# Ryan-D-Gast/ivp

Measured on AMD Instinct MI355X. Metric: accepted RK steps/sec (aggregate), batched CR3BP DOPRI5 @ rtol=1e-6, higher is better.
Workload: dtype f64; 1 GPU; C2: 100k independent 6-state CR3BP trajectories (perturbed Arenstorf orbits, one period), DOPRI5 rtol=1e-6 atol=1e-9; one step = whole batch integrated to t_end; trajectories_total=100000, trajectories_per_gpu=100000, fp_mode=strict, chunk_attempts=64, parallelism=dp1 (independent shards)

## Files before the change

ivp_amd/csrc/bdf_core.h:

```cpp
#pragma once
#ifndef __HIPCC_RTC__
#include "rk_core.h"
#endif

namespace IVP_NS {

constexpr int BDF_MAXO = 5;
#define IVP_BDF_ORDER_SHIFT 4
#define IVP_BDF_NEQ_SHIFT 8
#define IVP_BDF_LU_CURRENT 0x1000u
#define IVP_BDF_PENDING 0x2000u

#if defined(IVP_PHASE_PROF) && defined(__HIP_DEVICE_COMPILE__)
__device__ __forceinline__ unsigned long long *ivp_phase_lds()
{
    __shared__ unsigned long long t[18];
    return t;
}
__device__ __forceinline__ bool ivp_phase_leader()
{
    return __builtin_amdgcn_mbcnt_hi(__builtin_amdgcn_read_exec_hi(), __builtin_amdgcn_mbcnt_lo(__builtin_amdgcn_read_exec_lo(), 0u)) == 0u;
}
__device__ __forceinline__ void ivp_phase_mark(int k)
{
// ... 756 lines not shown
    a.hlamb[js] = S.pending_factor;
    a.bdf_piv[js] = S.piv;
    a.flags[js] = (S.flags & ~IVP_F_FIRSTOUT) | (L.flags & IVP_F_FIRSTOUT);
    a.status[js] = S.status;
    a.nfev[js] += S.d_nfev; a.njev[js] += S.d_njev; a.nlu[js] += S.d_nlu;
    a.nstep[js] += S.d_nstep; a.naccpt[js] += S.d_naccpt; a.nrejct[js] += S.d_nrejct;
    if (FULL) {
        a.next_idx[js] = L.next_idx; a.n_filled[js] = L.n_filled; a.n_log[js] = L.n_log;
        a.n_seg[js] = L.n_seg; a.t_last[js] = L.t_last;
    }
    status_out = S.status;
    return it;
}

template <class R, int FULL>
IVP_HD int32_t radau_init_body(const IvpKArgs &a, uint32_t j);
template <class R, int FULL>
IVP_HD uint32_t radau_chunk_body(const IvpKArgs &a, uint32_t j, int32_t &status_out);

template <int M, class R, int FULL>
IVP_HD int32_t any_init_body(const IvpKArgs &a, uint32_t j)
{
    if constexpr (M == M_BDF) return bdf_init_body<R, FULL>(a, j);
    else if constexpr (M == M_RADAU) return radau_init_body<R, FULL>(a, j);
    else return init_body<M, R, FULL>(a, j);
}
template <int M, class R, int FULL, bool CTL = false>
IVP_HD uint32_t any_chunk_body(const IvpKArgs &a, uint32_t j, int32_t &status_out)
{
    if constexpr (M == M_BDF) return bdf_chunk_body<R, FULL>(a, j, status_out);
    else if constexpr (M == M_RADAU) return radau_chunk_body<R, FULL>(a, j, status_out);
    else return chunk_body<M, R, FULL, CTL>(a, j, status_out);
}

}
```

ivp_amd/csrc/ivp_capi.cpp:

```cpp
#include "../../include/ivp_hip.h"

#include <hip/hip_runtime.h>

#include <algorithm>
#include <atomic>
#include <cmath>
#include <cstdarg>
#include <cstdio>
#include <cstdlib>
#include <cstring>
#include <string>
#include <thread>
#include <vector>

#include "ivp_jit.h"
#include "ivp_kargs.h"
#include "rk_launch.h"
#include "ivp_ctx.h"

using namespace ivp_host;

namespace {

struct RhsDim { int n, p; };
const RhsDim kRhsDims[IVP_RHS_BUILTIN_COUNT] = {{1, 1}, {2, 0}, {2, 1}, {6, 1}, {3, 3}, {3, 0}, {2, 0}, {2, 0}, {2, 0}, {3, 0}, {2, 1},
                                                {2, 0}, {2, 2}, {2, 0}, {2, 0}, {3, 0}};
const int kRhsEvents[IVP_RHS_BUILTIN_COUNT] = {0, 0, 0, 0, 0, 0, 0, 0, 0, 0, 0, 1, 1, 1, 3, 0};

#define IVP_MAX_GROUP_N 512
bool group_builtin(int rhs_id, int *n, int *p)
{
    switch (rhs_id) {
    case IVP_RHS_LINEAR_DECAY_100: *n = 100; *p = 0; return true;
    case IVP_RHS_HEAT1D_256: *n = 256; *p = 1; return true;
    case IVP_RHS_DENSE_64: *n = 64; *p = 1; return true;
    }
    return false;
}

struct MethodSettings { double uround, safety, scale_min, scale_max, beta; uint64_t nstiff; };
MethodSettings method_defaults(int method)
{
    if (method == IVP_DOP853) return {2.3e-16, 0.9, 0.333, 6.0, 0.0, 1000};
    if (method == IVP_DOPRI5) return {2.3e-16, 0.9, 0.2, 10.0, 0.04, 1000};
    return {2.3e-16, 0.9, 0.2, 10.0, 0.0, 1000};
}
MethodSettings settings_of(const ivp_options_t *opt)
{
    if (!opt->has_settings) return method_defaults(opt->method);
// ... 57 lines not shown
        } else if (opt->method == IVP_RK23) {
            if (opt->max_steps == 0) return fail(ctx, IVP_ERR_MUST_BE_POSITIVE, "max_steps must be positive");
            if (m.safety >= 1.0 || m.safety <= 1e-4) return fail(ctx, IVP_ERR_OUT_OF_RANGE, "safety_factor = %g outside (1e-4, 1)", m.safety);
            if (m.scale_min <= 0.0 || m.scale_max <= m.scale_min)
                return fail(ctx, IVP_ERR_INVALID_SCALE_FACTORS, "scale factors min = %g, max = %g", m.scale_min, m.scale_max);
        } else {
            return fail(ctx, IVP_ERR_BAD_ARGUMENT, "has_settings applies to RK23 / DOPRI5 / DOP853");
        }
    }
    if (opt->rtol_vec && opt->rtol_vec_len != n) return fail(ctx, IVP_ERR_TOLERANCE_SIZE_MISMATCH, "rtol: expected %d, got %d", n, opt->rtol_vec_len);
    if (opt->atol_vec && opt->atol_vec_len != n) return fail(ctx, IVP_ERR_TOLERANCE_SIZE_MISMATCH, "atol: expected %d, got %d", n, opt->atol_vec_len);
    if (opt->t_eval && opt->n_eval < 0) return fail(ctx, IVP_ERR_BAD_ARGUMENT, "negative n_eval");
    if (opt->t_eval && !opt->t_eval_offsets && opt->n_eval > 0x7FFFFFFFll) return fail(ctx, IVP_ERR_BAD_ARGUMENT, "n_eval too large");
    if (opt->fp_mode != IVP_FP_STRICT && opt->fp_mode != IVP_FP_FAST) return fail(ctx, IVP_ERR_BAD_ARGUMENT, "unknown fp_mode");
    if (opt->chunk_attempts < 0) return fail(ctx, IVP_ERR_BAD_ARGUMENT, "negative chunk_attempts");
    if (opt->variant < 0 || opt->variant > 3) return fail(ctx, IVP_ERR_BAD_ARGUMENT, "unknown kernel variant %d", opt->variant);
    *n_out = n;
    *p_out = p;
    return IVP_OK;
}
namespace {

struct Tune {
    size_t coop_cap_lanes = 0;
    uint32_t bulk_chunk = 64;
    int bdf_occ2 = -1;
    int window = 1;
    int launches_per_poll = 3;
    int launches_per_poll_set = 0;
    int lds_lu = 1;
    int defer_eval = 1;
    int defer_events = 1;
    int bdf_lpw = 0;
    Tune()
    {
        if (const char *e = getenv("IVP_TUNE_COOP_CAP_LANES")) coop_cap_lanes = (size_t)strtoull(e, nullptr, 10);
        if (const char *e = getenv("IVP_TUNE_BULK_CHUNK")) bulk_chunk = (uint32_t)std::max(1l, strtol(e, nullptr, 10));
        if (const char *e = getenv("IVP_TUNE_BDF_OCC2")) bdf_occ2 = (int)strtol(e, nullptr, 10);
        if (const char *e = getenv("IVP_TUNE_WINDOW")) window = (int)strtol(e, nullptr, 10);
        if (const char *e = getenv("IVP_TUNE_LDS_LU")) lds_lu = (int)strtol(e, nullptr, 10);
        if (const char *e = getenv("IVP_TUNE_DEFER_EVAL")) defer_eval = (int)strtol(e, nullptr, 10);
        if (const char *e = getenv("IVP_TUNE_DEFER_EVENTS")) defer_events = (int)strtol(e, nullptr, 10);
        if (const char *e = getenv("IVP_TUNE_BDF_LPW")) bdf_lpw = (int)std::min(64l, std::max(0l, strtol(e, nullptr, 10)));
        if (const char *e = getenv("IVP_TUNE_LAUNCHES_PER_POLL")) { launches_per_poll = (int)std::min(16l, std::max(1l, strtol(e, nullptr, 10))); launches_per_poll_set = 1; }
    }
};
const Tune &tune() { static const Tune t; return t; }
bool trace_launches() { static const bool on = getenv("IVP_TRACE_LAUNCHES") != nullptr; return on; }
size_t coop_cap_lanes(const ivp_ctx *ctx) { return tune().coop_cap_lanes ? tune().coop_cap_lanes : 2u * (size_t)ctx->one_wave_per_simd(); }

constexpr uint32_t kMaxRanSlots = 1u << 16;

hipEvent_t pend_event(ivp_ctx *ctx)
{
    ivp_ctx::Pending &P = ctx->pend;
    if (P.ev_used == ctx->events.size()) {
        hipEvent_t e;
        if (hipEventCreate(&e) != hipSuccess) return nullptr;
        ctx->events.push_back(e);
    }
    return ctx->events[P.ev_used++];
}

hipError_t pend_launch(ivp_ctx *ctx, int what, const IvpKArgs &ka, uint32_t lanes, bool use_hoist, bool use_coop)
{
    const ivp_ctx::Pending &P = ctx->pend;
    hipStream_t s = P.stream;
    const bool fast = P.fp_mode == IVP_FP_FAST;
    if (P.jit) return ivp_jit_launch(P.prob.jit, (use_coop && what == IVP_LAUNCH_CHUNK) ? IVP_LAUNCH_COOP : what, P.method, P.fp_mode, P.full, ka, lanes, s);
    if (P.group && P.method == IVP_RADAU) return ivp_launch_radau_group_strict(what, P.prob.rhs_id, P.full, ka, lanes, s);
    if (P.group) return (fast ? ivp_launch_group_fast : ivp_launch_group_strict)(what, P.method, P.prob.rhs_id, P.full, ka, lanes, s);
    if (P.method == IVP_RADAU) return ivp_launch_radau_strict(what, P.prob.rhs_id, P.full, ka, lanes, s);
    if (P.method == IVP_BDF) {
        const bool occ2 = what == IVP_LAUNCH_CHUNK && (lanes > ctx->one_wave_per_simd() || tune().bdf_occ2 == 1) && tune().bdf_occ2 != 0;
        if (occ2) return (fast ? ivp_launch_bdf_fast_occ2 : ivp_launch_bdf_strict_occ2)(what, P.prob.rhs_id, P.full, ka, lanes, s);
        return (fast ? ivp_launch_bdf_fast : ivp_launch_bdf_strict)(what, P.prob.rhs_id, P.full, ka, lanes, s);
// ... 13 lines not shown
        }                                                                                                       \
    } while (0)

int enqueue_round(ivp_ctx *ctx)
{
    ivp_ctx::Pending &P = ctx->pend;
    hipStream_t s = P.stream;
    const uint32_t kOneWavePerSimd = ctx->one_wave_per_simd();
    uint32_t *counts = (uint32_t *)ctx->counts.p;
    const uint32_t lanes = P.lanes;
    const bool profile = P.profile != 0;
    const bool fits_one_wave = (size_t)lanes * (P.group ? (P.jit ? (uint32_t)ivp_group_width(P.n) : (uint32_t)IVP_WAVE) : 1u) <= kOneWavePerSimd;
    const bool spec_ok = P.coop_ok && P.variant == 0 && P.adaptive && P.n >= 4 && !P.jit;
    bool use_hoist = !P.has_settings &&
                     (P.variant == 2 || (P.variant == 0 && (size_t)lanes <= 2 * (size_t)kOneWavePerSimd));
    const size_t coop_cap = coop_cap_lanes(ctx);
    const bool use_coop = P.coop_ok && (P.variant == 3 ||
                                        (P.variant == 0 && P.adaptive && P.n >= 4 && (size_t)lanes * 8u <= coop_cap));
    const bool tail = P.adaptive && (use_coop || (fits_one_wave && !spec_ok));
    int launches_per_sync = tail ? 1 : tune().launches_per_poll;
    uint32_t this_chunk = tail ? 1024u : P.chunk_now;
    if (P.lds_lu_ok && P.variant == 0 && !P.lu_probed && (size_t)lanes > 2u * (size_t)ctx->cus) {
        P.lu_probed = true;
        launches_per_sync = 1;
        this_chunk = 2u;
    }
    uint32_t lpw = 0;
    if ((P.method == IVP_BDF || P.method == IVP_RADAU) && !P.group) {
        const uint32_t cus = ctx->cus;
        const uint32_t want = tune().bdf_lpw > 0 ? (uint32_t)tune().bdf_lpw : std::max(1u, (lanes + cus - 1u) / cus);
        lpw = std::min(64u, want);
    }
    uint32_t window = 0;
    const bool alone = inflight_on(ctx->device).load(std::memory_order_relaxed) <= 1;
    if (tune().window && alone && P.adaptive && !P.group && !use_coop && !tail && lpw == 0 && P.method != IVP_BDF && P.method != IVP_RADAU && !P.has_events &&
        (P.n >= 4 || tune().window == 2)) {
        const uint32_t full = lanes / kOneWavePerSimd;
        if (full >= 1 && full < 4 && (uint64_t)lanes * 5u < (uint64_t)(full + 1u) * kOneWavePerSimd * 4u) window = full * kOneWavePerSimd;
        if (window) launches_per_sync = (int)(((uint64_t)launches_per_sync * lanes + window - 1u) / window);
        if (window && !P.has_settings && P.variant == 0 && (size_t)window <= 2 * (size_t)kOneWavePerSimd) use_hoist = true;
    }
    const bool paired = !tail && !use_coop && spec_ok;
    const uint32_t pair_threshold = (uint32_t)(coop_cap / 8u);
    if (paired && tune().launches_per_poll_set == 0) launches_per_sync += 1;
    auto ran_slot = [&]() -> uint32_t * {
        if (!profile || !paired || P.step_ev.size() >= kMaxRanSlots) return nullptr;
        return (uint32_t *)ctx->ran.p + P.step_ev.size();
    };
    for (int r = 0; r < launches_per_sync; ++r, ++P.c) {
        const uint64_t c = P.c;
        IvpKArgs ka = P.a;
        ka.chunk = this_chunk;
        ka.lpw = lpw;
        ka.window = window;
        ka.spec_min = (paired && c > 0) ? pair_threshold : 0u;
        ka.ran_out = ran_slot();
        ka.lds_lu = (P.lds_lu_ok && (P.variant == 2 || (size_t)lanes <= 2u * (size_t)ctx->cus || P.lu_dense)) ? 1u : 0u;
        if (P.band_lds) ka.lds_lu = 1u;
        if (c == 0) {
            ka.perm_in = nullptr;
            ka.count_in = nullptr;
        } else {
            ka.perm_in = (const uint32_t *)ctx->perm[(c - 1) & 1].p;
            ka.count_in = counts + ((c - 1) & 3);
        }
        ka.perm_out = (uint32_t *)ctx->perm[c & 1].p;
        ka.count_out = counts + (c & 3);
        ka.count_next = counts + ((c + 1) & 3);
        hipEvent_t e0 = nullptr, e1 = nullptr;
        if (profile) { e0 = pend_event(ctx); HIP_TRY(ctx, hipEventRecord(e0, s)); }
        LAUNCH_TRY(ctx, pend_launch(ctx, IVP_LAUNCH_CHUNK, ka, lanes, use_hoist, use_coop));
        if (profile) { e1 = pend_event(ctx); HIP_TRY(ctx, hipEventRecord(e1, s)); P.step_ev.emplace_back(e0, e1); P.step_is_coop.push_back((use_coop ? 1 : 0) | (ka.ran_out ? 2 : 0)); P.step_lanes.push_back(lanes); }
        if (!profile) { ctx->stats.launches += 1; if (use_coop) ctx->stats.coop_launches += 1; }
        if (paired && c > 0) {
            IvpKArgs kc = ka;
            kc.chunk = 1024u;
            kc.spec_min = 0u;
            kc.spec_cap = pair_threshold;
            kc.lpw = 0u;
            kc.window = 0u;
            kc.ran_out = ran_slot();
// ... 40 lines not shown
        P.sampled = true;
        LAUNCH_TRY(ctx, pend_launch(ctx, IVP_LAUNCH_EVENTS, P.a, (uint32_t)P.B, false, false));
        HIP_TRY(ctx, hipEventRecord(P.round_done, P.stream));
        return IVP_OK;
    }
    if (P.full == 3 && !P.sampled) {
        P.sampled = true;
        if (trace_launches() && P.profile) fprintf(stderr, "ivp launch sample  deferred t_eval sampling, %zu trajectories\n", P.B);
        const bool fast = P.fp_mode == IVP_FP_FAST;
        LAUNCH_TRY(ctx, (fast ? ivp_launch_fast : ivp_launch_strict)(IVP_LAUNCH_SAMPLE, P.method, P.prob.rhs_id, 3, P.a, (uint32_t)P.B, P.stream));
        HIP_TRY(ctx, hipEventRecord(P.round_done, P.stream));
        return IVP_OK;
    }
    set_active(ctx, false);
    *done = 1;
    if (P.paged) {
        ctx->log_state.overflow = (ctx->pinned[1] & 0x2u) != 0;
        ctx->log_state.valid = !ctx->log_state.overflow;
    }
    if (P.profile) {
        hipStream_t s = P.stream;
        hipEvent_t ev_end = pend_event(ctx);
        HIP_TRY(ctx, hipEventRecord(ev_end, s));
        HIP_TRY(ctx, hipEventSynchronize(ev_end));
        float ms = 0.f;
        HIP_TRY(ctx, hipEventElapsedTime(&ms, P.ev_t0, P.ev_init1));
        ctx->stats.init_kernel_ms = ms;
        std::vector<uint32_t> ran(std::min(P.step_ev.size(), (size_t)kMaxRanSlots), 1u);
        if (!ran.empty()) HIP_TRY(ctx, hipMemcpy(ran.data(), ctx->ran.p, ran.size() * sizeof(uint32_t), hipMemcpyDeviceToHost));
        for (size_t q = 0; q < P.step_ev.size(); ++q) {
            HIP_TRY(ctx, hipEventElapsedTime(&ms, P.step_ev[q].first, P.step_ev[q].second));
            const bool coop = (P.step_is_coop[q] & 1) != 0, flagged = (P.step_is_coop[q] & 2) != 0;
            const bool did = !flagged || q >= ran.size() || ran[q] != 0;
            if (trace_launches()) fprintf(stderr, "ivp launch %3zu  %-4s %-8s lanes<=%-8u %8.4f ms\n", q, coop ? "coop" : "bulk", did ? "ran" : "declined", P.step_lanes[q], ms);
            ctx->stats.step_kernel_ms += ms;
            if (coop) ctx->stats.coop_kernel_ms += ms;
            if (did) {
                ctx->stats.launches += 1;
                if (coop) ctx->stats.coop_launches += 1;
            } else {
                ctx->stats.declined_launches += 1;
                ctx->stats.declined_ms += ms;
                if (coop) { ctx->stats.declined_coop_launches += 1; ctx->stats.declined_coop_ms += ms; }
            }
        }
        HIP_TRY(ctx, hipEventElapsedTime(&ms, P.ev_t0, ev_end));
        ctx->stats.total_ms = ms;
        unsigned long long slots[2] = {0, 0};
        HIP_TRY(ctx, hipMemcpy(slots, ctx->slot.p, sizeof slots, hipMemcpyDeviceToHost));
        ctx->stats.lane_attempt_slots = slots[0];
        ctx->stats.lane_launches = slots[1];
        if (P.profile >= 2) {
            const size_t B = P.B;
            std::vector<uint64_t> tmp(B);
            HIP_TRY(ctx, hipMemcpy(tmp.data(), P.a.naccpt, sizeof(uint64_t) * B, hipMemcpyDeviceToHost));
            uint64_t acc = 0, att = 0;
            for (uint64_t v : tmp) acc += v;
            ctx->stats.total_accepted = acc;
            if (P.method == IVP_RK23) {
                HIP_TRY(ctx, hipMemcpy(tmp.data(), P.a.nrejct, sizeof(uint64_t) * B, hipMemcpyDeviceToHost));
                att = acc;
                for (uint64_t v : tmp) att += v;
            } else {
                HIP_TRY(ctx, hipMemcpy(tmp.data(), P.a.nstep, sizeof(uint64_t) * B, hipMemcpyDeviceToHost));
                for (uint64_t v : tmp) att += v;
            }
            ctx->stats.total_attempts = att;
// ... 1107 lines not shown
```

ivp_amd/csrc/ivp_kargs.h:

```cpp
#pragma once
#ifndef __HIPCC_RTC__
#include <stdint.h>
#endif

#define IVP_MAX_N 8
#define IVP_MAX_P 16
#define IVP_WAVE 64
#define IVP_RUNNING (-1)

#define IVP_F_LAST      0x1u
#define IVP_F_REJECT    0x2u
#define IVP_F_FIRSTOUT  0x4u
#define IVP_F_IASTI_SHIFT 4
#define IVP_F_NONSTIFF_SHIFT 8
#define IVP_F_STIFFCTR_SHIFT 12

struct IvpKArgs {
    uint32_t B;
    const double *y0;
    const double *params;
    const double *t0;
    const double *t1;
    uint32_t t0_stride;
    uint32_t t1_stride;
// ... 54 lines not shown
    const int32_t *ev_direction_dev;
    const uint32_t *ev_terminal_dev;
    uint32_t max_events;
    double *t_events;
    double *y_events;
    uint32_t *n_ev;
    double *prev_event;
    double *t_term;
    double min_step;
    int32_t has_min_step;
    double *bdf_d;
    double *bdf_jac;
    double *bdf_lu;
    uint32_t *bdf_piv;
    uint64_t *njev, *nlu;
    uint32_t *err_flag;
    unsigned long long *slot_counter;
    uint32_t spec_cap;
    uint32_t spec_min;
    uint32_t *ran_out;
    uint32_t lds_lu;
    uint32_t lpw;
    uint32_t *count_next;
    uint32_t window;
    double *def_rec;
    uint32_t def_cap;
    double *log_pool;
    unsigned long long log_region;
    uint32_t log_sub_mask;
    unsigned long long *log_alloc;
    double *evd_rec;
    uint32_t *evd_cnt;
    uint32_t evd_cap;
};
#define IVP_LOG_SLOTS 32u
#define IVP_LOG_HDR(cols) ((1u + 2u * (cols) + 15u) & ~15u)
#define IVP_LOG_GROUP(np1) ((np1) <= 9 ? 8u : 1u)
#define IVP_LOG_SUBPOOLS 64u
#define IVP_LOG_ALLOC_STRIDE 16u
#define IVP_NO_SEG 0xFFFFFFFFFFFFFFFFull
```

ivp_amd/csrc/rk_core.h:

```cpp
#pragma once
#ifndef __HIPCC_RTC__
#include <stdint.h>
#include <math.h>
#include "ivp_kargs.h"
#endif

#ifndef IVP_HD
#define IVP_HD __host__ __device__ __forceinline__
#endif
#ifndef IVP_FAST
#define IVP_FAST 0
#endif
#ifndef IVP_NS
#define IVP_NS ivp
#endif
#ifndef IVP_HOIST
#define IVP_HOIST 0
#endif
#if defined(__HIP_DEVICE_COMPILE__) && !IVP_HOIST
#define KC_SCOPE const uint64_t ivp_kz = IVP_NS::ivp_opaque_zero();
#define KC(c) IVP_NS::u2d(__builtin_bit_cast(uint64_t, (double)(c)) ^ ivp_kz)
#elif defined(__HIP_DEVICE_COMPILE__) && IVP_HOIST == 2
#define KC_SCOPE const uint64_t ivp_kz = 0;
#define KC(c) IVP_NS::u2d(__builtin_bit_cast(uint64_t, (double)(c)) ^ ivp_kz)
// ... 865 lines not shown
            a.log_alloc[(size_t)sub * IVP_LOG_ALLOC_STRIDE] = old + ((1ull << 40) | need);
#endif
            const unsigned long long used = old & ((1ull << 40) - 1ull), dir_idx = old >> 40;
            ok = used + need + dir_idx + 1u <= a.log_region;
            base = (unsigned long long)sub * a.log_region + used;
            if (ok && lane == first) {
                ((unsigned long long *)a.log_pool)[(size_t)(sub + 1u) * a.log_region - 1u - (size_t)dir_idx] =
                    (base << 8) | ((unsigned long long)(cols - 1u) << 2) | (unsigned long long)(arena - 1u);
                for (uint32_t q = 1; q < arena; ++q) *(uint32_t *)(a.log_pool + (size_t)(base + q * stride)) = 0u;
            }
        } else {
            ok = L.log_seg != IVP_NO_SEG;
            acols = (uint32_t)IVP_SEG_ACOLS(L.log_seg);
            base = IVP_SEG_BASE(L.log_seg) + ivp_log_page_doubles(acols, slots, np1);
        }
        if (!ok) {
            ivp_flag_error(a, IVP_ERRFLAG_LOG_OVERFLOW);
        } else {
            seg = ((uint64_t)base << 23) | ((uint64_t)(slots - 1u) << 18) | ((uint64_t)(acols - 1u) << 12) | ((uint64_t)(cols - 1u) << 6) | (uint64_t)col;
            if (lane == first) {
                uint32_t *ph = (uint32_t *)(a.log_pool + (size_t)base);
                ph[0] = cols;
                ph[1] = slots;
            }
            uint32_t *hdr = (uint32_t *)(a.log_pool + (size_t)base + 1u + 2u * (size_t)col);
            hdr[0] = j;
            hdr[1] = L.n_log;
            hdr[2] = 0u;
        }
    }
    L.log_seg = map_bcast64<MAP>(seg);
    L.log_bits = 0;
}
template <class MAP, int FULL, int N, int P>
IVP_HD void so_log_attempt(const IvpKArgs &a, uint32_t j, Lane<N, P> &L, uint32_t it)
{
    constexpr uint32_t kPerAttempt = FULL == 2 ? 1u : 2u, kAttempts = IVP_LOG_SLOTS / kPerAttempt;
    const uint32_t q = it & (kAttempts - 1u);
    if (q == 0u) {
        const uint32_t want = (a.chunk + kAttempts - 1u) / kAttempts;
        const uint32_t slots = want >= 2u ? IVP_LOG_SLOTS : (a.chunk * kPerAttempt < IVP_LOG_SLOTS ? a.chunk * kPerAttempt : IVP_LOG_SLOTS);
        so_log_open<MAP>(a, j, L, slots, it / kAttempts, want >= 4u ? 4u : (want >= 2u ? 2u : 1u));
    }
    L.log_slot = q * kPerAttempt;
}
template <int M, int N, int P, class MAP = IdMap<N>>
IVP_HD void so_push_log(const IvpKArgs &a, uint32_t j, Lane<N, P> &L, double t, const double *yv)
{
    const size_t B = a.B;
    if (a.log_pool != nullptr) {
        if (L.log_seg != IVP_NO_SEG) {
            constexpr size_t np1 = MAP::NT + 1, W = IVP_LOG_GROUP(np1);
            const size_t cols = IVP_SEG_COLS(L.log_seg), col = IVP_SEG_COL(L.log_seg), slots = IVP_SEG_SLOTS(L.log_seg);
            double *rec = a.log_pool + IVP_SEG_BASE(L.log_seg) + IVP_LOG_HDR(cols) + (((col / W) * slots + (size_t)L.log_slot) * W + (col % W)) * np1;
            if (MAP::leader()) rec[0] = t;
#pragma unroll
            for (int c = 0; c < N; ++c) if (MAP::own(c)) rec[1 + MAP::gi(c)] = yv[c];
            L.log_bits |= 1u << L.log_slot;
        }
        L.log_slot += 1;
    } else if (a.log_off != nullptr) {
        const unsigned long long lo = a.log_off[j], cap = a.log_off[j + 1] - lo;
        if (L.n_log < cap) {
            const size_t q = (size_t)(lo + L.n_log);
            a.t_log[q] = t;
#pragma unroll
            for (int c = 0; c < N; ++c) if (MAP::own(c)) a.y_log[q * MAP::NT + MAP::gi(c)] = yv[c];
        }
    } else if (L.n_log < a.max_log) {
        const size_t k = L.n_log;
        a.t_log[k * B + j] = t;
#pragma unroll
        for (int c = 0; c < N; ++c) if (MAP::own(c)) a.y_log[(k * MAP::NT + MAP::gi(c)) * B + j] = yv[c];
    }
// ... 1293 lines not shown
    R::ode(x + C3 * h, yt, k3, p);
#pragma unroll
    for (int i = 0; i < N; ++i) yt[i] = IVP_MA(y[i], h * 1.0, k3[i]);
    R::ode(x + 1.0 * h, yt, k4, p);
    const double xnew = x + h;
    {
        const double cB1 = KC(B1), cB2 = KC(B2), cB3 = KC(B3), cB4 = KC(B4);
#pragma unroll
        for (int i = 0; i < N; ++i) {
            yold[i] = y[i];
            L.y[i] = IVP_MA(y[i], h, IVP_LC(cB1, k1[i], cB2, k2[i], cB3, k3[i], cB4, k4[i]));
        }
    }
    R::ode(xnew, L.y, L.k1, p);
    L.x = xnew;
    L.d_nfev += 4;
    L.d_nstep += 1;
    if (FULL == 2) so_log_accepted<R>(a, j, L, xnew, L.y);
    if (FULL == 1) {
        double cont[4 * N];
#pragma unroll
        for (int i = 0; i < N; ++i) {
            cont[i] = yold[i];
            cont[N + i] = k4[i];
            cont[2 * N + i] = L.k1[i];
            cont[3 * N + i] = L.y[i];
        }
        if (solout_full<M_RK4, R>(a, j, L, x, xnew, L.y, cont, cont, h, x)) { L.status = 1; return false; }
    }
    if (last) { L.status = 0; return false; }
    return true;
}

template <int M, class R, int FULL, bool CTL = false>
IVP_HD uint32_t chunk_body(const IvpKArgs &a, uint32_t j, int32_t &status_out)
{
    Lane<R::N, R::P> L;
    lane_load<R>(a, j, L, M == M_RK23 || M == M_RK4, FULL);
#if defined(__HIP_DEVICE_COMPILE__) && IVP_HOIST >= 1
    L.kz = ivp_opaque_zero_v();
#else
    L.kz = 0;
#endif
    if (a.has_max_step) L.hmax = (M == M_DOPRI5) ? a.max_step : fabs(a.max_step);
    else L.hmax = fabs(L.xend - L.x0);
    if constexpr (HasInbandOde<R>::v) { L.inb_seed = R::inband_seed(L.p); L.inb_plain = false; }
    uint32_t it = 0;
    bool run = true;
    while (run && it < a.chunk) {
        if ((FULL == 1 || FULL == 2) && a.log_pool != nullptr) so_log_attempt<typename OutMap<R>::type, FULL>(a, j, L, it);
        if constexpr (M == M_DOPRI5) run = dopri5_attempt<R, FULL, CTL>(a, j, L);
        else if constexpr (M == M_DOP853) run = dop853_attempt<R, FULL, CTL>(a, j, L);
        else if constexpr (M == M_RK4) run = rk4_attempt<R, FULL>(a, j, L);
        else run = rk23_attempt<R, FULL, CTL>(a, j, L);
        ++it;
    }
    if ((FULL == 1 || FULL == 2) && a.log_pool != nullptr) so_log_flush<typename OutMap<R>::type>(a, L);
    uint32_t js = j;
    IVP_OPAQUE_V(js);
    lane_store<R>(a, js, L, FULL);
    status_out = L.status;
    return it;
}

}
```

ivp_amd/csrc/rk_global.h:

```cpp
#pragma once
#ifndef IVP_MIN_WAVES
#define IVP_MIN_WAVES 2
#endif
#ifndef IVP_BDF_MIN_WAVES
#define IVP_BDF_MIN_WAVES 1
#endif

namespace IVP_NS {

__device__ __forceinline__ uint32_t lane_id() { return __lane_id(); }

__device__ __forceinline__ void compact_append(const IvpKArgs &a, uint32_t j, bool still)
{
    const unsigned long long m = __ballot(still);
    if (m == 0ull) return;
    const uint32_t lane = lane_id();
    const uint32_t rank = __popcll(m & ((1ull << lane) - 1ull));
    const int leader = __ffsll((long long)m) - 1;
    uint32_t base = 0;
    if ((int)lane == leader) base = atomicAdd(a.count_out, (uint32_t)__popcll(m));
    base = __shfl(base, leader);
    if (still) a.perm_out[base + rank] = j;
}

// ... 44 lines not shown
    bool active = false;
    if (valid) {
        j = a.perm_in ? a.perm_in[i] : i;
        active = a.status[j] == IVP_RUNNING;
    }
    if (a.window && blockIdx.x * lpw >= a.window) {
        compact_append(a, j, active);
        return;
    }
    uint32_t it = 0;
    int32_t st = 0;
    if (active) it = any_chunk_body<M, R, FULL, CTL>(a, j, st);
    const bool still = active && st == IVP_RUNNING;
    compact_append(a, j, still);
    if (a.slot_counter) {
        uint32_t mx = it;
#pragma unroll
        for (int o = 32; o > 0; o >>= 1) mx = max(mx, (uint32_t)__shfl_xor((int)mx, o));
        const unsigned long long act = __ballot(active);
        if (lane_id() == 0) {
            atomicAdd(a.slot_counter, (unsigned long long)mx * IVP_WAVE);
            atomicAdd(a.slot_counter + 1, (unsigned long long)__popcll(act));
        }
    }
}

template <int M, class R, int FULL, bool CTL = false>
__global__ __launch_bounds__(IVP_WAVE, (M == M_BDF) ? IVP_BDF_MIN_WAVES : ((M == M_DOP853 && FULL == 1 && R::N >= 5) ? 1 : IVP_MIN_WAVES)) void chunk_kernel_t(const IvpKArgs a)
{
    chunk_kernel_body<M, R, FULL, CTL>(a);
}

}
```

ivp_amd/csrc/rk_kernels.hip:

```cpp
#include <hip/hip_runtime.h>

#define IVP_HD __host__ __device__ __forceinline__
#ifndef IVP_HOIST
#define IVP_HOIST 0
#endif
#if IVP_FAST && IVP_HOIST
#define IVP_NS ivp_fast_h
#define IVP_LAUNCH_NAME ivp_launch_fast_hoist
#elif IVP_FAST
#define IVP_NS ivp_fast
#define IVP_LAUNCH_NAME ivp_launch_fast
#elif IVP_HOIST
#define IVP_NS ivp_strict_h
#define IVP_LAUNCH_NAME ivp_launch_strict_hoist
#else
#define IVP_NS ivp_strict
#define IVP_LAUNCH_NAME ivp_launch_strict
#endif
#include "rk_core.h"
#include "bdf_core.h"
#include "rk_global.h"
#include "rk_launch.h"

namespace {

using namespace IVP_NS;

template <int M, class R, int FULL>
hipError_t launch_one(int what, const IvpKArgs &a, uint32_t lanes, hipStream_t s)
{
    const dim3 grid((lanes + IVP_WAVE - 1) / IVP_WAVE), block(IVP_WAVE);
    if (grid.x == 0) return hipSuccess;
    (void)hipGetLastError();
    if (what == IVP_LAUNCH_INIT) {
        hipLaunchKernelGGL((init_kernel_t<M, R, FULL>), grid, block, 0, s, a);
        return hipGetLastError();
    }
    constexpr bool kHasCtl = !IVP_HOIST && (M == M_RK23 || M == M_DOPRI5 || M == M_DOP853);
    if constexpr (kHasCtl) {
        if (a.has_ctl) {
            hipLaunchKernelGGL((chunk_kernel_t<M, R, FULL, true>), grid, block, 0, s, a);
            return hipGetLastError();
        }
    } else if (a.has_ctl) {
        return hipErrorInvalidValue;
    }
    hipLaunchKernelGGL((chunk_kernel_t<M, R, FULL>), grid, block, 0, s, a);
    return hipGetLastError();
}

template <int M, class R>
hipError_t launch_flavour(int what, int full, const IvpKArgs &a, uint32_t lanes, hipStream_t s)
{
    if constexpr (R::NE == 0 && M != M_RK4) {
        if (full == 2) return launch_one<M, R, 2>(what, a, lanes, s);
    }
    if constexpr (R::NE == 0 && M == M_DOP853) {
        if (full == 3) {
#if !IVP_HOIST
            if (what == IVP_LAUNCH_SAMPLE) {
                const dim3 grid((lanes + IVP_WAVE - 1) / IVP_WAVE, 8), block(IVP_WAVE);
                (void)hipGetLastError();
                hipLaunchKernelGGL((sample_kernel_t<R>), grid, block, 0, s, a);
                return hipGetLastError();
            }
#endif
            return launch_one<M, R, 3>(what, a, lanes, s);
        }
    }
// ... 52 lines not shown
```

ivp_amd/csrc/rk_launch.h:

```cpp
#pragma once
#include <hip/hip_runtime.h>
#include "ivp_kargs.h"

static inline int ivp_group_width(int n) { return n <= 16 ? 16 : (n <= 32 ? 32 : 64); }

enum { IVP_LAUNCH_INIT = 0, IVP_LAUNCH_CHUNK = 1, IVP_LAUNCH_COOP = 2 ,
       IVP_LAUNCH_SAMPLE = 3 ,
       IVP_LAUNCH_EVENTS = 4  };

hipError_t ivp_launch_strict(int what, int method, int rhs_id, int full, const IvpKArgs &a, uint32_t lanes, hipStream_t s);
hipError_t ivp_launch_strict_hoist(int what, int method, int rhs_id, int full, const IvpKArgs &a, uint32_t lanes, hipStream_t s);
hipError_t ivp_launch_fast_hoist(int what, int method, int rhs_id, int full, const IvpKArgs &a, uint32_t lanes, hipStream_t s);
hipError_t ivp_launch_fast(int what, int method, int rhs_id, int full, const IvpKArgs &a, uint32_t lanes, hipStream_t s);

hipError_t ivp_launch_group_strict(int what, int method, int rhs_id, int full, const IvpKArgs &a, uint32_t trajectories, hipStream_t s);
hipError_t ivp_launch_group_fast(int what, int method, int rhs_id, int full, const IvpKArgs &a, uint32_t trajectories, hipStream_t s);

hipError_t ivp_launch_coop_strict(int method, int rhs_id, int full, const IvpKArgs &a, uint32_t trajectories, hipStream_t s);
hipError_t ivp_launch_coop_fast(int method, int rhs_id, int full, const IvpKArgs &a, uint32_t trajectories, hipStream_t s);

hipError_t ivp_launch_bdf_strict(int what, int rhs_id, int full, const IvpKArgs &a, uint32_t lanes, hipStream_t s);
hipError_t ivp_launch_bdf_fast(int what, int rhs_id, int full, const IvpKArgs &a, uint32_t lanes, hipStream_t s);
hipError_t ivp_launch_bdf_strict_occ2(int what, int rhs_id, int full, const IvpKArgs &a, uint32_t lanes, hipStream_t s);
hipError_t ivp_launch_bdf_fast_occ2(int what, int rhs_id, int full, const IvpKArgs &a, uint32_t lanes, hipStream_t s);

hipError_t ivp_launch_radau_strict(int what, int rhs_id, int full, const IvpKArgs &a, uint32_t lanes, hipStream_t s);
hipError_t ivp_launch_radau_group_strict(int what, int rhs_id, int full, const IvpKArgs &a, uint32_t trajectories, hipStream_t s);
#define IVP_RADAU_MAX_N 64
```

Before: 8.393 billion steps/s.

## Add balanced work-splitting launch for partially filled windowed RK batches

Adds a balanced launch mode. When the lane count only partly fills a whole number of wave slots, the total attempt budget (wave-blocks times attempts) is split evenly into segments across a set of launches. Each wave block may run pieces of several trajectory blocks, which removes the tail imbalance where some SIMDs idle. The mode is limited to the CR3BP builtin with DOPRI5/DOP853 and no controller. It adds more launches and extra per-piece state reloads, and changes when compaction happens.

```diff
diff --git a/ivp_amd/csrc/bdf_core.h b/ivp_amd/csrc/bdf_core.h
--- a/ivp_amd/csrc/bdf_core.h
+++ b/ivp_amd/csrc/bdf_core.h
@@ -812,5 +812,11 @@
     else if constexpr (M == M_RADAU) return radau_chunk_body<R, FULL>(a, j, status_out);
     else return chunk_body<M, R, FULL, CTL>(a, j, status_out);
 }
-
-}
+template <int M, class R, int FULL, bool CTL = false>
+IVP_HD uint32_t any_chunk_body(const IvpKArgs &a, uint32_t j, int32_t &status_out, uint32_t attempts)
+{
+    static_assert(M != M_BDF && M != M_RADAU, "explicit RK methods only");
+    return chunk_body<M, R, FULL, CTL, true>(a, j, status_out, attempts);
+}
+
+}
diff --git a/ivp_amd/csrc/ivp_balance.h b/ivp_amd/csrc/ivp_balance.h
--- /dev/null
+++ b/ivp_amd/csrc/ivp_balance.h
@@ -0,0 +1,80 @@
+#pragma once
+#ifndef __HIPCC_RTC__
+#include <stdint.h>
+#endif
+
+#ifndef IVP_BAL_HD
+#if defined(__HIPCC__) || defined(__HIPCC_RTC__)
+#define IVP_BAL_HD __host__ __device__ inline
+#else
+#define IVP_BAL_HD inline
+#endif
+#endif
+
+struct IvpBalancePlan {
+    uint32_t L;
+    uint32_t q;
+    uint32_t W;
+};
+
+constexpr IVP_BAL_HD uint32_t ivp_balance_window(uint32_t lanes, uint32_t S)
+{
+    const uint64_t one = (uint64_t)S * 64u;
+    if (one == 0u || one > 0xFFFFFFFFull) return 0u;
+    const uint64_t full = lanes / one;
+    if (full >= 1u && full < 4u && (uint64_t)lanes * 5u < (full + 1u) * one * 4u) return (uint32_t)(full * one);
+    return 0u;
+}
+
+constexpr IVP_BAL_HD IvpBalancePlan ivp_balance_plan(uint32_t lanes, uint32_t R, uint32_t S, uint32_t chunk)
+{
+    IvpBalancePlan none = {0u, 0u, 0u};
+    if (S == 0u || chunk == 0u || R < chunk || R > 0xFFFFu) return none;
+    if (ivp_balance_window(lanes, S) == 0u) return none;
+    const uint64_t nb = ((uint64_t)lanes + 63u) / 64u, total = nb * R;
+    const uint64_t lower = (total + (uint64_t)S * chunk - 1u) / ((uint64_t)S * chunk);
+    for (uint64_t L = lower; L <= 2u * lower && L <= 255u; ++L) {
+        const uint64_t q = (total + (uint64_t)S * L - 1u) / ((uint64_t)S * L);
+        if ((R + q - 1u) / q + 1u <= L) {
+            const uint64_t segs = (total + q - 1u) / q;
+            IvpBalancePlan p = {(uint32_t)L, (uint32_t)q, (uint32_t)((segs + L - 1u) / L)};
+            return p;
+        }
+    }
+    return none;
+}
+
+struct IvpBalancePiece {
+    uint32_t b, n;
+    bool last;
+};
+
+constexpr IVP_BAL_HD uint32_t ivp_balance_last_launch(uint32_t b, uint32_t R, uint32_t q, uint32_t L)
+{
+    const uint64_t s_lo = (uint64_t)b * R / q, s_hi = ((uint64_t)(b + 1u) * R - 1u) / q;
+    if (s_lo / L != s_hi / L) return L - 1u;
+    return (uint32_t)(s_hi % L);
+}
+
+constexpr IVP_BAL_HD uint32_t ivp_balance_pieces(uint32_t w, uint32_t l, uint32_t nb, uint32_t R, uint32_t q, uint32_t L, IvpBalancePiece out[2])
+{
+    const uint64_t total = (uint64_t)nb * R;
+    uint64_t u = ((uint64_t)w * L + l) * q;
+    const uint64_t uend = u + q < total ? u + q : total;
+    uint32_t k = 0;
+    while (u < uend && k < 2u) {
+        const uint64_t b = u / R, bend = (b + 1u) * R;
+        const uint64_t n = (uend < bend ? uend : bend) - u;
+        out[k].b = (uint32_t)b;
+        out[k].n = (uint32_t)n;
+        out[k].last = ivp_balance_last_launch((uint32_t)b, R, q, L) == l;
+        u += n;
+        ++k;
+    }
+    return k;
+}
+
+constexpr IVP_BAL_HD uint32_t ivp_balance_pack(uint32_t R, uint32_t L, uint32_t l) { return (R << 16) | (L << 8) | l; }
+constexpr IVP_BAL_HD uint32_t ivp_balance_R(uint32_t word) { return word >> 16; }
+constexpr IVP_BAL_HD uint32_t ivp_balance_L(uint32_t word) { return (word >> 8) & 0xFFu; }
+constexpr IVP_BAL_HD uint32_t ivp_balance_l(uint32_t word) { return word & 0xFFu; }
diff --git a/ivp_amd/csrc/ivp_capi.cpp b/ivp_amd/csrc/ivp_capi.cpp
--- a/ivp_amd/csrc/ivp_capi.cpp
+++ b/ivp_amd/csrc/ivp_capi.cpp
@@ -15,6 +15,7 @@
 
 #include "ivp_jit.h"
 #include "ivp_kargs.h"
+#include "ivp_balance.h"
 #include "rk_launch.h"
 #include "ivp_ctx.h"
 
@@ -138,6 +139,8 @@
     int defer_eval = 1;
     int defer_events = 1;
     int bdf_lpw = 0;
+    int balance = 1;
+    uint32_t balance_slots = 0;
     Tune()
     {
         if (const char *e = getenv("IVP_TUNE_COOP_CAP_LANES")) coop_cap_lanes = (size_t)strtoull(e, nullptr, 10);
@@ -148,6 +151,8 @@
         if (const char *e = getenv("IVP_TUNE_DEFER_EVAL")) defer_eval = (int)strtol(e, nullptr, 10);
         if (const char *e = getenv("IVP_TUNE_DEFER_EVENTS")) defer_events = (int)strtol(e, nullptr, 10);
         if (const char *e = getenv("IVP_TUNE_BDF_LPW")) bdf_lpw = (int)std::min(64l, std::max(0l, strtol(e, nullptr, 10)));
+        if (const char *e = getenv("IVP_TUNE_BALANCE")) balance = (int)strtol(e, nullptr, 10);
+        if (const char *e = getenv("IVP_TUNE_BALANCE_SLOTS")) balance_slots = (uint32_t)std::min(1l << 20, std::max(0l, strtol(e, nullptr, 10)));
         if (const char *e = getenv("IVP_TUNE_LAUNCHES_PER_POLL")) { launches_per_poll = (int)std::min(16l, std::max(1l, strtol(e, nullptr, 10))); launches_per_poll_set = 1; }
     }
 };
@@ -227,13 +232,16 @@
         lpw = std::min(64u, want);
     }
     uint32_t window = 0;
+    const uint32_t slots = tune().balance_slots ? tune().balance_slots : kOneWavePerSimd / (uint32_t)IVP_WAVE;
+    IvpBalancePlan plan = {0u, 0u, 0u};
     const bool alone = inflight_on(ctx->device).load(std::memory_order_relaxed) <= 1;
     if (tune().window && alone && P.adaptive && !P.group && !use_coop && !tail && lpw == 0 && P.method != IVP_BDF && P.method != IVP_RADAU && !P.has_events &&
         (P.n >= 4 || tune().window == 2)) {
-        const uint32_t full = lanes / kOneWavePerSimd;
-        if (full >= 1 && full < 4 && (uint64_t)lanes * 5u < (uint64_t)(full + 1u) * kOneWavePerSimd * 4u) window = full * kOneWavePerSimd;
+        window = ivp_balance_window(lanes, slots);
+        if (window && tune().balance && !P.jit && ivp_has_balanced(P.method, P.prob.rhs_id, P.full, P.a.has_ctl))
+            plan = ivp_balance_plan(lanes, (uint32_t)tune().launches_per_poll * this_chunk, slots, this_chunk);
         if (window) launches_per_sync = (int)(((uint64_t)launches_per_sync * lanes + window - 1u) / window);
-        if (window && !P.has_settings && P.variant == 0 && (size_t)window <= 2 * (size_t)kOneWavePerSimd) use_hoist = true;
+        if (window && !P.has_settings && P.variant == 0 && ((size_t)window <= 2 * (size_t)slots * IVP_WAVE || plan.L)) use_hoist = true;
     }
     const bool paired = !tail && !use_coop && spec_ok;
     const uint32_t pair_threshold = (uint32_t)(coop_cap / 8u);
@@ -242,6 +250,32 @@
         if (!profile || !paired || P.step_ev.size() >= kMaxRanSlots) return nullptr;
         return (uint32_t *)ctx->ran.p + P.step_ev.size();
     };
+    if (plan.L) {
+        const uint64_t c = P.c;
+        const uint32_t R = (uint32_t)tune().launches_per_poll * this_chunk;
+        for (uint32_t l = 0; l < plan.L; ++l) {
+            IvpKArgs ka = P.a;
+            ka.chunk = plan.q;
+            ka.balance = ivp_balance_pack(R, plan.L, l);
+            ka.lpw = 0u;
+            ka.window = 0u;
+            ka.spec_min = 0u;
+            ka.ran_out = nullptr;
+            ka.lds_lu = 0u;
+            ka.perm_in = c == 0 ? nullptr : (const uint32_t *)ctx->perm[(c - 1) & 1].p;
+            ka.count_in = c == 0 ? nullptr : counts + ((c - 1) & 3);
+            ka.perm_out = (uint32_t *)ctx->perm[c & 1].p;
+            ka.count_out = counts + (c & 3);
+            ka.count_next = counts + ((c + 1) & 3);
+            hipEvent_t e0 = nullptr, e1 = nullptr;
+            if (profile) { e0 = pend_event(ctx); HIP_TRY(ctx, hipEventRecord(e0, s)); }
+            LAUNCH_TRY(ctx, pend_launch(ctx, IVP_LAUNCH_BALANCED, ka, plan.W * (uint32_t)IVP_WAVE, use_hoist, false));
+            if (profile) { e1 = pend_event(ctx); HIP_TRY(ctx, hipEventRecord(e1, s)); P.step_ev.emplace_back(e0, e1); P.step_is_coop.push_back(4); P.step_lanes.push_back(lanes); }
+            if (!profile) ctx->stats.launches += 1;
+        }
+        ++P.c;
+        launches_per_sync = (paired && tune().launches_per_poll_set == 0) ? 1 : 0;
+    }
     for (int r = 0; r < launches_per_sync; ++r, ++P.c) {
         const uint64_t c = P.c;
         IvpKArgs ka = P.a;
@@ -348,7 +382,7 @@
             HIP_TRY(ctx, hipEventElapsedTime(&ms, P.step_ev[q].first, P.step_ev[q].second));
             const bool coop = (P.step_is_coop[q] & 1) != 0, flagged = (P.step_is_coop[q] & 2) != 0;
             const bool did = !flagged || q >= ran.size() || ran[q] != 0;
-            if (trace_launches()) fprintf(stderr, "ivp launch %3zu  %-4s %-8s lanes<=%-8u %8.4f ms\n", q, coop ? "coop" : "bulk", did ? "ran" : "declined", P.step_lanes[q], ms);
+            if (trace_launches()) fprintf(stderr, "ivp launch %3zu  %-4s %-8s lanes<=%-8u %8.4f ms\n", q, coop ? "coop" : ((P.step_is_coop[q] & 4) ? "bal" : "bulk"), did ? "ran" : "declined", P.step_lanes[q], ms);
             ctx->stats.step_kernel_ms += ms;
             if (coop) ctx->stats.coop_kernel_ms += ms;
             if (did) {
diff --git a/ivp_amd/csrc/ivp_kargs.h b/ivp_amd/csrc/ivp_kargs.h
--- a/ivp_amd/csrc/ivp_kargs.h
+++ b/ivp_amd/csrc/ivp_kargs.h
@@ -110,6 +110,7 @@
     double *evd_rec;
     uint32_t *evd_cnt;
     uint32_t evd_cap;
+    uint32_t balance;
 };
 #define IVP_LOG_SLOTS 32u
 #define IVP_LOG_HDR(cols) ((1u + 2u * (cols) + 15u) & ~15u)
diff --git a/ivp_amd/csrc/rk_core.h b/ivp_amd/csrc/rk_core.h
--- a/ivp_amd/csrc/rk_core.h
+++ b/ivp_amd/csrc/rk_core.h
@@ -921,14 +921,14 @@
     L.log_seg = map_bcast64<MAP>(seg);
     L.log_bits = 0;
 }
-template <class MAP, int FULL, int N, int P>
-IVP_HD void so_log_attempt(const IvpKArgs &a, uint32_t j, Lane<N, P> &L, uint32_t it)
+template <class MAP, int FULL, bool PIECE = false, int N, int P>
+IVP_HD void so_log_attempt(const IvpKArgs &a, uint32_t j, Lane<N, P> &L, uint32_t it, uint32_t piece = 0)
 {
     constexpr uint32_t kPerAttempt = FULL == 2 ? 1u : 2u, kAttempts = IVP_LOG_SLOTS / kPerAttempt;
     const uint32_t q = it & (kAttempts - 1u);
     if (q == 0u) {
-        const uint32_t want = (a.chunk + kAttempts - 1u) / kAttempts;
-        const uint32_t slots = want >= 2u ? IVP_LOG_SLOTS : (a.chunk * kPerAttempt < IVP_LOG_SLOTS ? a.chunk * kPerAttempt : IVP_LOG_SLOTS);
+        const uint32_t want = ((PIECE ? piece : a.chunk) + kAttempts - 1u) / kAttempts;
+        const uint32_t slots = want >= 2u ? IVP_LOG_SLOTS : ((PIECE ? piece : a.chunk) * kPerAttempt < IVP_LOG_SLOTS ? (PIECE ? piece : a.chunk) * kPerAttempt : IVP_LOG_SLOTS);
         so_log_open<MAP>(a, j, L, slots, it / kAttempts, want >= 4u ? 4u : (want >= 2u ? 2u : 1u));
     }
     L.log_slot = q * kPerAttempt;
@@ -2288,8 +2288,8 @@
     return true;
 }
 
-template <int M, class R, int FULL, bool CTL = false>
-IVP_HD uint32_t chunk_body(const IvpKArgs &a, uint32_t j, int32_t &status_out)
+template <int M, class R, int FULL, bool CTL = false, bool PIECE = false>
+IVP_HD uint32_t chunk_body(const IvpKArgs &a, uint32_t j, int32_t &status_out, uint32_t piece = 0)
 {
     Lane<R::N, R::P> L;
     lane_load<R>(a, j, L, M == M_RK23 || M == M_RK4, FULL);
@@ -2303,8 +2303,8 @@
     if constexpr (HasInbandOde<R>::v) { L.inb_seed = R::inband_seed(L.p); L.inb_plain = false; }
     uint32_t it = 0;
     bool run = true;
-    while (run && it < a.chunk) {
-        if ((FULL == 1 || FULL == 2) && a.log_pool != nullptr) so_log_attempt<typename OutMap<R>::type, FULL>(a, j, L, it);
+    while (run && it < (PIECE ? piece : a.chunk)) {
+        if ((FULL == 1 || FULL == 2) && a.log_pool != nullptr) so_log_attempt<typename OutMap<R>::type, FULL, PIECE>(a, j, L, it, piece);
         if constexpr (M == M_DOPRI5) run = dopri5_attempt<R, FULL, CTL>(a, j, L);
         else if constexpr (M == M_DOP853) run = dop853_attempt<R, FULL, CTL>(a, j, L);
         else if constexpr (M == M_RK4) run = rk4_attempt<R, FULL>(a, j, L);
diff --git a/ivp_amd/csrc/rk_global.h b/ivp_amd/csrc/rk_global.h
--- a/ivp_amd/csrc/rk_global.h
+++ b/ivp_amd/csrc/rk_global.h
@@ -100,3 +100,52 @@
 }
 
 }
+
+#ifndef __HIPCC_RTC__
+#include "ivp_balance.h"
+namespace IVP_NS {
+
+template <int M, class R, int FULL>
+__global__ __launch_bounds__(IVP_WAVE, IVP_MIN_WAVES) void balanced_chunk_kernel_t(const IvpKArgs a)
+{
+    const uint32_t count = a.perm_in ? *a.count_in : a.B;
+    if (a.count_next && blockIdx.x == 0 && threadIdx.x == 0) *a.count_next = 0u;
+    const uint32_t Rr = ivp_balance_R(a.balance), L = ivp_balance_L(a.balance), l = ivp_balance_l(a.balance), q = a.chunk;
+    const uint32_t nb = (count + (uint32_t)IVP_WAVE - 1u) / (uint32_t)IVP_WAVE;
+    if (Rr == 0u || L == 0u || q == 0u) return;
+    const uint64_t total = (uint64_t)nb * Rr;
+    uint64_t u = ((uint64_t)blockIdx.x * L + l) * q;
+    const uint64_t uend = u + q < total ? u + q : total;
+#pragma unroll 1
+    while (u < uend) {
+        const uint32_t b = (uint32_t)(u / Rr);
+        const uint64_t bend = (uint64_t)(b + 1u) * Rr;
+        const uint32_t n = (uint32_t)((uend < bend ? uend : bend) - u);
+        const bool last = ivp_balance_last_launch(b, Rr, q, L) == l;
+        u += n;
+        const uint32_t i = b * (uint32_t)IVP_WAVE + threadIdx.x;
+        uint32_t j = 0;
+        bool active = false;
+        if (i < count) {
+            j = a.perm_in ? a.perm_in[i] : i;
+            active = a.status[j] == IVP_RUNNING;
+        }
+        uint32_t it = 0;
+        int32_t st = 0;
+        if (active) it = any_chunk_body<M, R, FULL>(a, j, st, n);
+        if (last) compact_append(a, j, active && st == IVP_RUNNING);
+        if (a.slot_counter) {
+            uint32_t mx = it;
+#pragma unroll
+            for (int o = 32; o > 0; o >>= 1) mx = max(mx, (uint32_t)__shfl_xor((int)mx, o));
+            const unsigned long long act = __ballot(active);
+            if (lane_id() == 0) {
+                atomicAdd(a.slot_counter, (unsigned long long)mx * IVP_WAVE);
+                atomicAdd(a.slot_counter + 1, (unsigned long long)__popcll(act));
+            }
+        }
+    }
+}
+
+}
+#endif
diff --git a/ivp_amd/csrc/rk_kernels.hip b/ivp_amd/csrc/rk_kernels.hip
--- a/ivp_amd/csrc/rk_kernels.hip
+++ b/ivp_amd/csrc/rk_kernels.hip
@@ -35,6 +35,14 @@
     if (what == IVP_LAUNCH_INIT) {
         hipLaunchKernelGGL((init_kernel_t<M, R, FULL>), grid, block, 0, s, a);
         return hipGetLastError();
+    }
+    if (what == IVP_LAUNCH_BALANCED) {
+        if constexpr ((M == M_DOPRI5 || M == M_DOP853) && (FULL == 0 || FULL == 2) && R::N >= 4 && R::NE == 0) {
+            if (a.has_ctl || a.balance == 0u) return hipErrorInvalidValue;
+            hipLaunchKernelGGL((balanced_chunk_kernel_t<M, R, FULL>), grid, block, 0, s, a);
+            return hipGetLastError();
+        }
+        return hipErrorInvalidValue;
     }
     constexpr bool kHasCtl = !IVP_HOIST && (M == M_RK23 || M == M_DOPRI5 || M == M_DOP853);
     if constexpr (kHasCtl) {
diff --git a/ivp_amd/csrc/rk_launch.h b/ivp_amd/csrc/rk_launch.h
--- a/ivp_amd/csrc/rk_launch.h
+++ b/ivp_amd/csrc/rk_launch.h
@@ -6,7 +6,13 @@
 
 enum { IVP_LAUNCH_INIT = 0, IVP_LAUNCH_CHUNK = 1, IVP_LAUNCH_COOP = 2 ,
        IVP_LAUNCH_SAMPLE = 3 ,
-       IVP_LAUNCH_EVENTS = 4  };
+       IVP_LAUNCH_EVENTS = 4 ,
+       IVP_LAUNCH_BALANCED = 5  };
+
+static inline bool ivp_has_balanced(int method, int rhs_id, int full, int has_ctl)
+{
+    return (method == 1 || method == 2) && (full == 0 || full == 2) && !has_ctl && rhs_id == 3;
+}
 
 hipError_t ivp_launch_strict(int what, int method, int rhs_id, int full, const IvpKArgs &a, uint32_t lanes, hipStream_t s);
 hipError_t ivp_launch_strict_hoist(int what, int method, int rhs_id, int full, const IvpKArgs &a, uint32_t lanes, hipStream_t s);
```

Result: faster. 8.611 billion steps/s (median of 6 runs) (+2.6%).
